# opendilab/DI-engine

Hardware: NVIDIA H100
Metric: learner transitions/sec (GAE+ppo_error fwd+bwd, T=128 x B=4096 per GPU) (higher is better)
Workload: dtype f32

## Files before the change

### di-engine_b200/csrc/colws.cu

```cuda
#include "../../include/b200rl.h"
#include "fused_args.cuh"

namespace b200rl {

constexpr int CW_CW = 8;
constexpr int CW_CT = CW_CW * 32;
constexpr int CW_THREADS = CW_CT + 64;
constexpr int CW_TC = 16;
constexpr int CW_R = CW_CT / CW_TC;
constexpr int CW_MAX_STAGES = 4;
constexpr int CW_RAW_ARR = CW_R * CW_TC * 4;
constexpr int CW_RAW_BYTES = 5 * CW_RAW_ARR;

#define CW_TRACE(slot)                                                                                   \
    do {                                                                                                 \
        if (f.trace) reinterpret_cast<unsigned long long*>(ws + 65536)[blockIdx.x * 32 + (slot)] = gtimer(); \
    } while (0)

struct CwItem {
    long long tile;
    long long q;
};

__host__ __device__ inline int cw_stage_bytes(int N, bool has_pre, bool has_w) {
    return (CW_CT * ((has_pre ? 3 : 2) * N * 4 + 8 + 12 + (has_w ? 4 : 0)) + 127) & ~127;
}

template <int NC, bool GRADS>
__global__ void __launch_bounds__(CW_THREADS, 2) gae_ppo_ws_kernel(FusedArgs f, float* ws, int n_stages) {
    asm volatile("griddepcontrol.launch_dependents;" ::: "memory");
    extern __shared__ __align__(128) unsigned char smem[];
    const PpoArgs& a = f.p;
    const int N = NC ? NC : a.N;
    const int tid = threadIdx.x, wid = tid >> 5, lane = tid & 31;
    const bool has_pre = a.logit_pre != nullptr, has_w = a.weight != nullptr;
    PpoTileLayout L;
    {
        L.logit_bytes = CW_CT * N * 4;
        int o = L.logit_bytes;
        L.off_old = o; o += L.logit_bytes;
        L.off_pre = o; if (has_pre) o += L.logit_bytes;
        L.off_act = o; o += CW_CT * 8;
        L.off_vn = o; o += CW_CT * 4;
        L.off_vo = o; o += CW_CT * 4;
        L.off_adv = 0;
        L.off_ret = o; o += CW_CT * 4;
        L.off_w = o; if (has_w) o += CW_CT * 4;
        L.stage_bytes = (o + 127) & ~127;
        L.tx_bytes = o;
    }
    const int S = n_stages;
    unsigned char* raw = smem + S * L.stage_bytes;
    auto advr = reinterpret_cast<float (*)[CW_R][CW_TC]>(raw + 2 * CW_RAW_BYTES);
    auto fbuf = reinterpret_cast<float (*)[CW_TC]>(reinterpret_cast<unsigned char*>(advr) + CW_MAX_STAGES * CW_RAW_ARR);
    uint64_t* bars = reinterpret_cast<uint64_t*>(reinterpret_cast<unsigned char*>(fbuf) + CW_RAW_ARR);
    uint64_t* full = bars;
    uint64_t* done = bars + CW_MAX_STAGES;
    uint64_t* adv_ready = bars + 2 * CW_MAX_STAGES;

    const long long T = f.T, B = f.B;
    const long long n_tiles = (B + CW_TC - 1) / CW_TC;
    const long long n_chunks = (T + CW_R - 1) / CW_R;
    const bool has_done = f.done != nullptr, has_traj = f.traj != nullptr;

    if (tid == 0) {
        CW_TRACE(0);
        for (int s = 0; s < CW_MAX_STAGES; ++s) {
            mbar_init(&full[s], 32);
            mbar_init(&done[s], CW_CW);
            mbar_init(&adv_ready[s], 1);
        }
        mbar_fence_init();
    }
    asm volatile("griddepcontrol.wait;" ::: "memory");
    __syncthreads();
    if (f.x_mailboxes && blockIdx.x == 0 && wid < 6) {
        XchgArgs x{f.x_mailboxes, f.x_seq, f.x_out_mean, f.x_rank, f.x_world};
        p2p_pipeline_warp(x, wid);
    }

    auto item_valid = [&](const CwItem& it) { return it.tile < n_tiles; };
    auto item_next = [&](CwItem& it) {
        if (++it.q >= n_chunks) {
            it.q = 0;
            it.tile += gridDim.x;
        }
    };
    const CwItem first{(long long)blockIdx.x, 0};
    float acc[6] = {0.f, 0.f, 0.f, 0.f, 0.f, 0.f};

    if (wid == CW_CW) {
        auto rows_of = [&](unsigned char* dst, const void* src, long long t0, long long c0, int esz, int jmin, int W) {
            const int P = CW_TC * esz / 16, Pv = W * esz / 16;
            const unsigned char* g = reinterpret_cast<const unsigned char*>(src) + (t0 * B + c0) * esz;
            const long long rstride = B * esz;
            const int n = CW_R * P;
#pragma unroll 4
            for (int p = lane; p < n; p += 32) {
                const int row = p / P, o = p - row * P;
                if (row >= jmin && o < Pv) cpa16(dst + p * 16, g + row * rstride + o * 16);
            }
        };
        CwItem it = first;
        int s = 0, ph = 0;
        for (int j = 0; item_valid(it); ++j) {
            if (j >= S) mbar_wait(&done[s], (uint32_t)(ph ^ 1));
            if (lane == 0 && j < 6) CW_TRACE(20 + 2 * j);
            const long long c0 = it.tile * CW_TC;
            const long long t0 = T - (it.q + 1) * CW_R;
            const int jmin = t0 < 0 ? (int)-t0 : 0;
            const int W = (int)((B - c0) < CW_TC ? (B - c0) : CW_TC);
            unsigned char* st = smem + s * L.stage_bytes;
            if (jmin == 0 && W == CW_TC && j == 0) {
                const uint32_t sb = smem_u32(st);
                const long long e0 = t0 * B + c0;
                const long long ls = B * N * 4;
                if (N & 1) {
                    warp_copy_rows<4, CW_R, NC>(sb, a.logit_new + e0 * N, ls, N, lane);
                    warp_copy_rows<4, CW_R, NC>(sb + L.off_old, a.logit_old + e0 * N, ls, N, lane);
                    if (has_pre) warp_copy_rows<4, CW_R, NC>(sb + L.off_pre, a.logit_pre + e0 * N, ls, N, lane);
                    warp_copy_rows<4, CW_R, 2>(sb + L.off_act, a.action + e0, B * 8, 2, lane);
                } else {
                    warp_copy_rows<8, CW_R, NC / 2>(sb, a.logit_new + e0 * N, ls, N / 2, lane);
                    warp_copy_rows<8, CW_R, NC / 2>(sb + L.off_old, a.logit_old + e0 * N, ls, N / 2, lane);
                    if (has_pre) warp_copy_rows<8, CW_R, NC / 2>(sb + L.off_pre, a.logit_pre + e0 * N, ls, N / 2, lane);
                    warp_copy_rows<8, CW_R, 1>(sb + L.off_act, a.action + e0, B * 8, 1, lane);
                }
                warp_copy_rows<4, CW_R, 1>(sb + L.off_vn, a.value_new + e0, B * 4, 1, lane);
                warp_copy_rows<4, CW_R, 1>(sb + L.off_vo, a.value_old + e0, B * 4, 1, lane);
                warp_copy_rows<4, CW_R, 1>(sb + L.off_ret, a.ret + e0, B * 4, 1, lane);
                if (has_w) warp_copy_rows<4, CW_R, 1>(sb + L.off_w, a.weight + e0, B * 4, 1, lane);
            } else {
                rows_of(st, a.logit_new, t0, c0, N * 4, jmin, W);
                rows_of(st + L.off_old, a.logit_old, t0, c0, N * 4, jmin, W);
                if (has_pre) rows_of(st + L.off_pre, a.logit_pre, t0, c0, N * 4, jmin, W);
                rows_of(st + L.off_act, a.action, t0, c0, 8, jmin, W);
                rows_of(st + L.off_vn, a.value_new, t0, c0, 4, jmin, W);
                rows_of(st + L.off_vo, a.value_old, t0, c0, 4, jmin, W);
                rows_of(st + L.off_ret, a.ret, t0, c0, 4, jmin, W);
                if (has_w) rows_of(st + L.off_w, a.weight, t0, c0, 4, jmin, W);
            }
            cpa_mbar_arrive(&full[s]);
            if (lane == 0 && j < 6) CW_TRACE(21 + 2 * j);
            if (++s == S) { s = 0; ph ^= 1; }
            item_next(it);
        }
    } else if (wid == CW_CW + 1) {
        auto issue_raw = [&](const CwItem& it, int slot) {
            const long long c0 = it.tile * CW_TC;
            const long long t0 = T - (it.q + 1) * CW_R;
            const int W = (int)((B - c0) < CW_TC ? (B - c0) : CW_TC);
            unsigned char* dst = raw + slot * CW_RAW_BYTES;
#pragma unroll
            for (int k = 0; k < 2; ++k) {
                const int p = lane + 32 * k;
                const int row = p >> 2, o = p & 3;
                if (t0 + row >= 0 && o * 4 < W) {
                    const long long off = (t0 + row) * B + c0 + o * 4;
                    cpa16(dst + p * 16, f.value + off);
                    cpa16(dst + CW_RAW_ARR + p * 16, f.next_value + off);
                    cpa16(dst + 2 * CW_RAW_ARR + p * 16, f.reward + off);
                    if (has_done) cpa16(dst + 3 * CW_RAW_ARR + p * 16, f.done + off);
                    if (has_traj) cpa16(dst + 4 * CW_RAW_ARR + p * 16, f.traj + off);
                }
            }
        };
        CwItem it = first, pf = first;
        for (int k = 0; k < 2; ++k) {
            if (item_valid(pf)) {
                issue_raw(pf, k);
                item_next(pf);
            }
            cpa_commit();
        }
        float carry = 0.f;
        int s = 0, ph = 0;
        for (int j = 0; item_valid(it); ++j) {
            const long long c0 = it.tile * CW_TC;
            const long long t0 = T - (it.q + 1) * CW_R;
            const int slot = j & 1;
            if (it.q == 0) carry = 0.f;
            cpa_wait<1>();
            __syncwarp();
            if (j >= S) mbar_wait(&done[s], (uint32_t)(ph ^ 1));
            float (*ab)[CW_TC] = advr[s];
            const float* rv = reinterpret_cast<const float*>(raw + slot * CW_RAW_BYTES);
            const float* rn = rv + CW_R * CW_TC;
            const float* rr = rn + CW_R * CW_TC;
            const float* rd = rr + CW_R * CW_TC;
            const float* rt = rd + CW_R * CW_TC;
            const int cq = (lane & 3) * 4;
#pragma unroll
            for (int p = 0; p < CW_R / 8; ++p) {
                const int jj = p * 8 + (lane >> 2);
                const long long t = t0 + jj;
                if (t >= 0 && c0 + cq < B) {
                    const int o = jj * CW_TC + cq;
                    const float4 v4 = *reinterpret_cast<const float4*>(rv + o);
                    const float4 n4 = *reinterpret_cast<const float4*>(rn + o);
                    const float4 r4 = *reinterpret_cast<const float4*>(rr + o);
                    const float4 d4 = has_done ? *reinterpret_cast<const float4*>(rd + o) : make_float4(0.f, 0.f, 0.f, 0.f);
                    const float4 t4 = has_traj ? *reinterpret_cast<const float4*>(rt + o) : d4;
                    float vv[4] = {v4.x, v4.y, v4.z, v4.w}, nn[4] = {n4.x, n4.y, n4.z, n4.w};
                    float rw[4] = {r4.x, r4.y, r4.z, r4.w}, dd[4] = {d4.x, d4.y, d4.z, d4.w};
                    float tt[4] = {t4.x, t4.y, t4.z, t4.w};
                    float de[4], fa[4];
                    bool changed = false;
#pragma unroll
                    for (int k = 0; k < 4; ++k) {
                        if (has_done) {
                            changed |= (dd[k] != 0.f);
                            nn[k] = fmul(nn[k], fsub(1.f, dd[k]));
                        }
                        de[k] = fsub(fadd(rw[k], fmul(f.gamma, nn[k])), vv[k]);
                        fa[k] = fmul(f.gl, fsub(1.f, tt[k]));
                    }
                    *reinterpret_cast<float4*>(&ab[jj][cq]) = make_float4(de[0], de[1], de[2], de[3]);
                    *reinterpret_cast<float4*>(&fbuf[jj][cq]) = make_float4(fa[0], fa[1], fa[2], fa[3]);
                    if (changed && f.mask_inplace)
                        *reinterpret_cast<float4*>(f.next_value + t * B + c0 + cq) =
                            make_float4(nn[0], nn[1], nn[2], nn[3]);
                }
            }
            __syncwarp();
            if (item_valid(pf)) {
                issue_raw(pf, slot);
                item_next(pf);
            }
            cpa_commit();
            if (lane < CW_TC && c0 + lane < B) {
                if (t0 >= 0) {
                    float d[CW_R], g[CW_R];
#pragma unroll
                    for (int k = 0; k < CW_R; ++k) {
                        d[k] = ab[CW_R - 1 - k][lane];
                        g[k] = fbuf[CW_R - 1 - k][lane];
                    }
#pragma unroll
                    for (int k = 0; k < CW_R; ++k) {
                        carry = fadd(d[k], fmul(g[k], carry));
                        ab[CW_R - 1 - k][lane] = carry;
                    }
                } else {
                    for (int jj = CW_R - 1; jj >= 0 && t0 + jj >= 0; --jj) {
                        carry = fadd(ab[jj][lane], fmul(fbuf[jj][lane], carry));
                        ab[jj][lane] = carry;
                    }
                }
            }
            __syncwarp();
            if (lane == 0) {
                mbar_arrive(&adv_ready[s]);
                if (j == 0) CW_TRACE(19);
            }
#pragma unroll
            for (int k = 0; k < 2; ++k) {
                const int p = lane + 32 * k;
                const int row = p >> 2, o = (p & 3) * 4;
                if (t0 + row >= 0 && c0 + o < B)
                    stg_stream4(reinterpret_cast<float4*>(a.adv_out + (t0 + row) * B + c0 + o),
                                *reinterpret_cast<const float4*>(&ab[row][o]));
            }
            if (++s == S) { s = 0; ph ^= 1; }
            item_next(it);
        }
        cpa_wait<0>();
    } else {
        PpoUpstream up{0.f, 0.f, 0.f, 0.f, 1.f / (float)a.S};
        if (GRADS) {
            up.g_pol = a.g_policy ? *a.g_policy : 0.f;
            up.g_val = a.g_value ? *a.g_value : 0.f;
            up.g_ent = a.g_entropy ? *a.g_entropy : 0.f;
            up.g_kl = (a.g_kl && has_pre) ? *a.g_kl : 0.f;
            if (a.g_used && blockIdx.x == 0 && tid == 0) {
                a.g_used[0] = up.g_pol; a.g_used[1] = up.g_val; a.g_used[2] = up.g_ent; a.g_used[3] = up.g_kl;
            }
        }
        const int jj = tid / CW_TC, c = tid % CW_TC;
        CwItem it = first;
        int s = 0, ph = 0;
        for (int j = 0; item_valid(it); ++j) {
            const long long c0 = it.tile * CW_TC;
            const long long t = T - (it.q + 1) * CW_R + jj;
            unsigned char* st = smem + s * L.stage_bytes;
            mbar_wait(&full[s], (uint32_t)ph);
            if (tid == 0 && j < 6) CW_TRACE(1 + 3 * j);
            mbar_wait(&adv_ready[s], (uint32_t)ph);
            if (tid == 0 && j < 6) CW_TRACE(2 + 3 * j);
            if (t >= 0 && c0 + c < B) {
                const long long g = t * B + c0 + c;
                float* grow = GRADS ? a.grad_logit + g * N : nullptr;
                float* gval = GRADS ? a.grad_value + g : nullptr;
                ppo_row_compute_to<NC, true, GRADS>(a, L, st, tid, N, advr[s][jj][c], grow, gval, up, acc);
            }
            __syncwarp();
            if (lane == 0) mbar_arrive(&done[s]);
            if (tid == 0 && j < 6) CW_TRACE(3 + 3 * j);
            if (++s == S) { s = 0; ph ^= 1; }
            item_next(it);
        }
    }
    grid_store_partials<6, CW_THREADS>(acc, ws);
}

static size_t cw_smem(int N, bool has_pre, bool has_w, int stages) {
    return (size_t)stages * cw_stage_bytes(N, has_pre, has_w) + 2 * CW_RAW_BYTES + CW_MAX_STAGES * CW_RAW_ARR + CW_RAW_ARR +
           3 * CW_MAX_STAGES * sizeof(uint64_t) + 32;
}

static int cw_pick_stages(const FusedArgs& f) {
    const PpoArgs& a = f.p;
    for (int s = CW_MAX_STAGES; s >= 2; --s)
        if (cw_smem(a.N, a.logit_pre != nullptr, a.weight != nullptr, s) <= 112 * 1024) return s;
    return 0;
}

bool colws_ok(const FusedArgs& f) {
    const PpoArgs& a = f.p;
    const bool al = aligned16(a.logit_new) && aligned16(a.logit_old) && (!a.logit_pre || aligned16(a.logit_pre)) &&
                    aligned16(a.action) && aligned16(a.value_new) && aligned16(a.value_old) && aligned16(a.ret) &&
                    (!a.weight || aligned16(a.weight)) && (!a.grad_logit || aligned16(a.grad_logit)) &&
                    (!a.grad_value || aligned16(a.grad_value)) && aligned16(f.value) && aligned16(f.next_value) &&
                    aligned16(f.reward) && aligned16(a.adv) && (!f.done || aligned16(f.done)) &&
                    (!f.traj || aligned16(f.traj));
    return al && a.N >= 1 && a.N <= 32 && f.T >= 1 && f.B >= 4 && (f.B % 4) == 0 && f.T * f.B == a.S &&
           cw_pick_stages(f) >= 2;
}

template <int NC, bool GRADS>
static int launch_ws(const FusedArgs& f, float* out, float* ws, size_t ws_bytes, cudaStream_t st) {
    const PpoArgs& a = f.p;
    const int stages = cw_pick_stages(f);
    const size_t smem = cw_smem(a.N, a.logit_pre != nullptr, a.weight != nullptr, stages);
    constexpr auto kern = gae_ppo_ws_kernel<NC, GRADS>;
    int sm_count, per_sm;
    if (int rc = resident_ctas<kern>(CW_THREADS, smem, sm_count, per_sm)) return rc;
    const long long n_tiles = (f.B + CW_TC - 1) / CW_TC;
    long long grid = (long long)sm_count * per_sm;
    if (grid > n_tiles) grid = n_tiles;
    if (ws_bytes < WS_MIN_BYTES || !ws_partials_fit((long long)(grid * 6), ws_bytes))
        return B200RL_ERR_WORKSPACE;
    if (int rc = launch_k(kern, (int)grid, CW_THREADS, smem, st, f, ws, stages)) return rc;
    FinalizeArgs fa = ppo_finalize_args(a.S, a.logit_pre != nullptr, (int)grid);
    fa.x.mailboxes = f.x_mailboxes; fa.x.state = f.x_seq; fa.x.out_mean = f.x_out_mean; fa.x.rank = f.x_rank;
    fa.x.world = f.x_world;
    return launch_finalize(ws, out, fa, st);
}

template <bool GRADS>
static int dispatch_ws(const FusedArgs& f, float* out, float* ws, size_t ws_bytes, cudaStream_t st) {
    return with_nc(f.p.N, [&](auto nc) { return launch_ws<nc, GRADS>(f, out, ws, ws_bytes, st); });
}

int launch_colws(const FusedArgs& f, bool grads, float* out, float* ws, size_t ws_bytes, cudaStream_t st) {
    return grads ? dispatch_ws<true>(f, out, ws, ws_bytes, st) : dispatch_ws<false>(f, out, ws, ws_bytes, st);
}

}
```

Before: 17.76 billion.

## Add 32-column tile geometry with one CTA per SM and L2 prefetch of first chunk

Templates the column-tiled warp-specialized GAE+PPO kernel on tile width, adding a 32-column variant (8 rows per chunk, up to 8 stages, one CTA per SM with a 224KB smem budget) picked when B is large enough and at least 6 stages fit. Each CTA also issues bulk L2 prefetches for its first chunk's rows before griddepcontrol.wait, to overlap the first loads with the previous kernel's tail. Tracing is made a compile-time template flag with more slots. The wider tiles are meant to give full 128B row segments and deeper pipelining, at the cost of halving resident CTAs and shortening the per-chunk scan length.

```diff
diff --git a/di-engine_b200/csrc/colws.cu b/di-engine_b200/csrc/colws.cu
--- a/di-engine_b200/csrc/colws.cu
+++ b/di-engine_b200/csrc/colws.cu
@@ -6,15 +6,38 @@
 constexpr int CW_CW = 8;
 constexpr int CW_CT = CW_CW * 32;
 constexpr int CW_THREADS = CW_CT + 64;
-constexpr int CW_TC = 16;
-constexpr int CW_R = CW_CT / CW_TC;
-constexpr int CW_MAX_STAGES = 4;
-constexpr int CW_RAW_ARR = CW_R * CW_TC * 4;
+constexpr int CW_RAW_ARR = CW_CT * 4;
 constexpr int CW_RAW_BYTES = 5 * CW_RAW_ARR;
 
-#define CW_TRACE(slot)                                                                                   \
-    do {                                                                                                 \
-        if (f.trace) reinterpret_cast<unsigned long long*>(ws + 65536)[blockIdx.x * 32 + (slot)] = gtimer(); \
+template <int TC>
+struct CwGeo {
+    static constexpr int R = CW_CT / TC;
+    static constexpr int CPS = TC == 32 ? 1 : 2;
+    static constexpr int MAX_STAGES = TC == 32 ? 8 : 4;
+    static constexpr int SMEM_BUDGET = CPS == 1 ? 224 * 1024 : 112 * 1024;
+    static constexpr int PR = TC / 4;
+};
+
+constexpr int CW_PF = 1;
+__device__ __forceinline__ void prefetch_l2(const void* p, uint32_t bytes) {
+    asm volatile("cp.async.bulk.prefetch.L2.global [%0], %1;" ::"l"(p), "r"(bytes) : "memory");
+}
+
+constexpr int CW_TRACE_CTAS = 512;
+constexpr int CW_TRACE_SLOTS = 64;
+#define CW_TRACE(slot)                                                                                                  \
+    do {                                                                                                                \
+        if (TRACE && blockIdx.x < CW_TRACE_CTAS)                                                                        \
+            reinterpret_cast<unsigned long long*>(ws + 65536)[(blockIdx.x * 2 + (f.trace - 1)) * CW_TRACE_SLOTS + (slot)] = \
+                gtimer();                                                                                               \
+    } while (0)
+__device__ __forceinline__ int cw_trace_k(int j, int nj) { return j < 4 ? j : (j >= nj - 2 && nj > 4) ? 4 + j - (nj - 2) : -1; }
+#define CW_TRACE_CHUNK(first, stride)                           \
+    do {                                                        \
+        if (TRACE) {                                            \
+            const int tk_ = cw_trace_k(j, s_nj);                \
+            if (tk_ >= 0) CW_TRACE((first) + (stride) * tk_);   \
+        }                                                       \
     } while (0)
 
 struct CwItem {
@@ -26,8 +49,10 @@
     return (CW_CT * ((has_pre ? 3 : 2) * N * 4 + 8 + 12 + (has_w ? 4 : 0)) + 127) & ~127;
 }
 
-template <int NC, bool GRADS>
-__global__ void __launch_bounds__(CW_THREADS, 2) gae_ppo_ws_kernel(FusedArgs f, float* ws, int n_stages) {
+template <int NC, bool GRADS, int TC, bool TRACE>
+__global__ void __launch_bounds__(CW_THREADS, CwGeo<TC>::CPS) gae_ppo_ws_kernel(FusedArgs f, float* ws, int n_stages) {
+    using G = CwGeo<TC>;
+    constexpr int R = G::R, PR = G::PR;
     asm volatile("griddepcontrol.launch_dependents;" ::: "memory");
     extern __shared__ __align__(128) unsigned char smem[];
     const PpoArgs& a = f.p;
@@ -51,28 +76,58 @@
     }
     const int S = n_stages;
     unsigned char* raw = smem + S * L.stage_bytes;
-    auto advr = reinterpret_cast<float (*)[CW_R][CW_TC]>(raw + 2 * CW_RAW_BYTES);
-    auto fbuf = reinterpret_cast<float (*)[CW_TC]>(reinterpret_cast<unsigned char*>(advr) + CW_MAX_STAGES * CW_RAW_ARR);
+    auto advr = reinterpret_cast<float (*)[R][TC]>(raw + 2 * CW_RAW_BYTES);
+    auto fbuf = reinterpret_cast<float (*)[TC]>(reinterpret_cast<unsigned char*>(advr) + G::MAX_STAGES * CW_RAW_ARR);
     uint64_t* bars = reinterpret_cast<uint64_t*>(reinterpret_cast<unsigned char*>(fbuf) + CW_RAW_ARR);
     uint64_t* full = bars;
-    uint64_t* done = bars + CW_MAX_STAGES;
-    uint64_t* adv_ready = bars + 2 * CW_MAX_STAGES;
+    uint64_t* done = bars + G::MAX_STAGES;
+    uint64_t* adv_ready = bars + 2 * G::MAX_STAGES;
 
     const long long T = f.T, B = f.B;
-    const long long n_tiles = (B + CW_TC - 1) / CW_TC;
-    const long long n_chunks = (T + CW_R - 1) / CW_R;
+    const long long n_tiles = (B + TC - 1) / TC;
+    const long long n_chunks = (T + R - 1) / R;
     const bool has_done = f.done != nullptr, has_traj = f.traj != nullptr;
+    __shared__ int s_nj;
 
     if (tid == 0) {
         CW_TRACE(0);
-        for (int s = 0; s < CW_MAX_STAGES; ++s) {
+        if (TRACE) s_nj = (int)(n_chunks * ((n_tiles - blockIdx.x + gridDim.x - 1) / gridDim.x));
+        for (int s = 0; s < G::MAX_STAGES; ++s) {
             mbar_init(&full[s], 32);
             mbar_init(&done[s], CW_CW);
             mbar_init(&adv_ready[s], 1);
         }
         mbar_fence_init();
     }
+    {
+        const long long c0 = (long long)blockIdx.x * TC;
+        const long long rows = T < (long long)CW_PF * R ? T : (long long)CW_PF * R;
+        const int W = (int)((B - c0) < TC ? (B - c0) : TC);
+        for (int i = tid; i < 13 * rows; i += CW_THREADS) {
+            const int k = (int)(i / rows);
+            const long long t = T - rows + (i - k * rows);
+            const void* p = nullptr;
+            int esz = 4;
+            switch (k) {
+                case 0: p = a.logit_new; esz = N * 4; break;
+                case 1: p = a.logit_old; esz = N * 4; break;
+                case 2: p = a.logit_pre; esz = N * 4; break;
+                case 3: p = a.action; esz = 8; break;
+                case 4: p = a.value_new; break;
+                case 5: p = a.value_old; break;
+                case 6: p = a.ret; break;
+                case 7: p = a.weight; break;
+                case 8: p = f.value; break;
+                case 9: p = f.next_value; break;
+                case 10: p = f.reward; break;
+                case 11: p = f.done; break;
+                default: p = f.traj; break;
+            }
+            if (p) prefetch_l2(reinterpret_cast<const unsigned char*>(p) + (t * B + c0) * esz, (uint32_t)(W * esz));
+        }
+    }
     asm volatile("griddepcontrol.wait;" ::: "memory");
+    if (tid == 0) CW_TRACE(1);
     __syncthreads();
     if (f.x_mailboxes && blockIdx.x == 0 && wid < 6) {
         XchgArgs x{f.x_mailboxes, f.x_seq, f.x_out_mean, f.x_rank, f.x_world};
@@ -91,10 +146,10 @@
 
     if (wid == CW_CW) {
         auto rows_of = [&](unsigned char* dst, const void* src, long long t0, long long c0, int esz, int jmin, int W) {
-            const int P = CW_TC * esz / 16, Pv = W * esz / 16;
+            const int P = TC * esz / 16, Pv = W * esz / 16;
             const unsigned char* g = reinterpret_cast<const unsigned char*>(src) + (t0 * B + c0) * esz;
             const long long rstride = B * esz;
-            const int n = CW_R * P;
+            const int n = R * P;
 #pragma unroll 4
             for (int p = lane; p < n; p += 32) {
                 const int row = p / P, o = p - row * P;
@@ -105,31 +160,32 @@
         int s = 0, ph = 0;
         for (int j = 0; item_valid(it); ++j) {
             if (j >= S) mbar_wait(&done[s], (uint32_t)(ph ^ 1));
-            if (lane == 0 && j < 6) CW_TRACE(20 + 2 * j);
-            const long long c0 = it.tile * CW_TC;
-            const long long t0 = T - (it.q + 1) * CW_R;
+            if (lane == 0) CW_TRACE_CHUNK(24, 2);
+            const long long c0 = it.tile * TC;
+            const long long t0 = T - (it.q + 1) * R;
             const int jmin = t0 < 0 ? (int)-t0 : 0;
-            const int W = (int)((B - c0) < CW_TC ? (B - c0) : CW_TC);
+            const int W = (int)((B - c0) < TC ? (B - c0) : TC);
             unsigned char* st = smem + s * L.stage_bytes;
-            if (jmin == 0 && W == CW_TC && j == 0) {
+            if (jmin == 0 && W == TC && j == 0) {
                 const uint32_t sb = smem_u32(st);
                 const long long e0 = t0 * B + c0;
                 const long long ls = B * N * 4;
-                if (N & 1) {
-                    warp_copy_rows<4, CW_R, NC>(sb, a.logit_new + e0 * N, ls, N, lane);
-                    warp_copy_rows<4, CW_R, NC>(sb + L.off_old, a.logit_old + e0 * N, ls, N, lane);
-                    if (has_pre) warp_copy_rows<4, CW_R, NC>(sb + L.off_pre, a.logit_pre + e0 * N, ls, N, lane);
-                    warp_copy_rows<4, CW_R, 2>(sb + L.off_act, a.action + e0, B * 8, 2, lane);
+                if (TC == 16 && (N & 1)) {
+                    warp_copy_rows<4, R, NC>(sb, a.logit_new + e0 * N, ls, N, lane);
+                    warp_copy_rows<4, R, NC>(sb + L.off_old, a.logit_old + e0 * N, ls, N, lane);
+                    if (has_pre) warp_copy_rows<4, R, NC>(sb + L.off_pre, a.logit_pre + e0 * N, ls, N, lane);
+                    warp_copy_rows<4, R, 2>(sb + L.off_act, a.action + e0, B * 8, 2, lane);
                 } else {
-                    warp_copy_rows<8, CW_R, NC / 2>(sb, a.logit_new + e0 * N, ls, N / 2, lane);
-                    warp_copy_rows<8, CW_R, NC / 2>(sb + L.off_old, a.logit_old + e0 * N, ls, N / 2, lane);
-                    if (has_pre) warp_copy_rows<8, CW_R, NC / 2>(sb + L.off_pre, a.logit_pre + e0 * N, ls, N / 2, lane);
-                    warp_copy_rows<8, CW_R, 1>(sb + L.off_act, a.action + e0, B * 8, 1, lane);
+                    constexpr int LPG = NC * TC / 32;
+                    warp_copy_rows<8, R, LPG>(sb, a.logit_new + e0 * N, ls, N * TC / 32, lane);
+                    warp_copy_rows<8, R, LPG>(sb + L.off_old, a.logit_old + e0 * N, ls, N * TC / 32, lane);
+                    if (has_pre) warp_copy_rows<8, R, LPG>(sb + L.off_pre, a.logit_pre + e0 * N, ls, N * TC / 32, lane);
+                    warp_copy_rows<8, R, TC / 16>(sb + L.off_act, a.action + e0, B * 8, TC / 16, lane);
                 }
-                warp_copy_rows<4, CW_R, 1>(sb + L.off_vn, a.value_new + e0, B * 4, 1, lane);
-                warp_copy_rows<4, CW_R, 1>(sb + L.off_vo, a.value_old + e0, B * 4, 1, lane);
-                warp_copy_rows<4, CW_R, 1>(sb + L.off_ret, a.ret + e0, B * 4, 1, lane);
-                if (has_w) warp_copy_rows<4, CW_R, 1>(sb + L.off_w, a.weight + e0, B * 4, 1, lane);
+                warp_copy_rows<PR, R, 1>(sb + L.off_vn, a.value_new + e0, B * 4, 1, lane);
+                warp_copy_rows<PR, R, 1>(sb + L.off_vo, a.value_old + e0, B * 4, 1, lane);
+                warp_copy_rows<PR, R, 1>(sb + L.off_ret, a.ret + e0, B * 4, 1, lane);
+                if (has_w) warp_copy_rows<PR, R, 1>(sb + L.off_w, a.weight + e0, B * 4, 1, lane);
             } else {
                 rows_of(st, a.logit_new, t0, c0, N * 4, jmin, W);
                 rows_of(st + L.off_old, a.logit_old, t0, c0, N * 4, jmin, W);
@@ -141,20 +197,20 @@
                 if (has_w) rows_of(st + L.off_w, a.weight, t0, c0, 4, jmin, W);
             }
             cpa_mbar_arrive(&full[s]);
-            if (lane == 0 && j < 6) CW_TRACE(21 + 2 * j);
+            if (lane == 0) CW_TRACE_CHUNK(25, 2);
             if (++s == S) { s = 0; ph ^= 1; }
             item_next(it);
         }
     } else if (wid == CW_CW + 1) {
         auto issue_raw = [&](const CwItem& it, int slot) {
-            const long long c0 = it.tile * CW_TC;
-            const long long t0 = T - (it.q + 1) * CW_R;
-            const int W = (int)((B - c0) < CW_TC ? (B - c0) : CW_TC);
+            const long long c0 = it.tile * TC;
+            const long long t0 = T - (it.q + 1) * R;
+            const int W = (int)((B - c0) < TC ? (B - c0) : TC);
             unsigned char* dst = raw + slot * CW_RAW_BYTES;
 #pragma unroll
             for (int k = 0; k < 2; ++k) {
                 const int p = lane + 32 * k;
-                const int row = p >> 2, o = p & 3;
+                const int row = p / PR, o = p % PR;
                 if (t0 + row >= 0 && o * 4 < W) {
                     const long long off = (t0 + row) * B + c0 + o * 4;
                     cpa16(dst + p * 16, f.value + off);
@@ -176,26 +232,26 @@
         float carry = 0.f;
         int s = 0, ph = 0;
         for (int j = 0; item_valid(it); ++j) {
-            const long long c0 = it.tile * CW_TC;
-            const long long t0 = T - (it.q + 1) * CW_R;
+            const long long c0 = it.tile * TC;
+            const long long t0 = T - (it.q + 1) * R;
             const int slot = j & 1;
             if (it.q == 0) carry = 0.f;
             cpa_wait<1>();
             __syncwarp();
             if (j >= S) mbar_wait(&done[s], (uint32_t)(ph ^ 1));
-            float (*ab)[CW_TC] = advr[s];
+            float (*ab)[TC] = advr[s];
             const float* rv = reinterpret_cast<const float*>(raw + slot * CW_RAW_BYTES);
-            const float* rn = rv + CW_R * CW_TC;
-            const float* rr = rn + CW_R * CW_TC;
-            const float* rd = rr + CW_R * CW_TC;
-            const float* rt = rd + CW_R * CW_TC;
-            const int cq = (lane & 3) * 4;
-#pragma unroll
-            for (int p = 0; p < CW_R / 8; ++p) {
-                const int jj = p * 8 + (lane >> 2);
+            const float* rn = rv + CW_CT;
+            const float* rr = rn + CW_CT;
+            const float* rd = rr + CW_CT;
+            const float* rt = rd + CW_CT;
+#pragma unroll
+            for (int p = 0; p < 2; ++p) {
+                const int q = lane + 32 * p;
+                const int jj = q / PR, cq = (q % PR) * 4;
                 const long long t = t0 + jj;
                 if (t >= 0 && c0 + cq < B) {
-                    const int o = jj * CW_TC + cq;
+                    const int o = jj * TC + cq;
                     const float4 v4 = *reinterpret_cast<const float4*>(rv + o);
                     const float4 n4 = *reinterpret_cast<const float4*>(rn + o);
                     const float4 r4 = *reinterpret_cast<const float4*>(rr + o);
@@ -228,21 +284,21 @@
                 item_next(pf);
             }
             cpa_commit();
-            if (lane < CW_TC && c0 + lane < B) {
+            if (lane < TC && c0 + lane < B) {
                 if (t0 >= 0) {
-                    float d[CW_R], g[CW_R];
-#pragma unroll
-                    for (int k = 0; k < CW_R; ++k) {
-                        d[k] = ab[CW_R - 1 - k][lane];
-                        g[k] = fbuf[CW_R - 1 - k][lane];
+                    float d[R], g[R];
+#pragma unroll
+                    for (int k = 0; k < R; ++k) {
+                        d[k] = ab[R - 1 - k][lane];
+                        g[k] = fbuf[R - 1 - k][lane];
                     }
 #pragma unroll
-                    for (int k = 0; k < CW_R; ++k) {
+                    for (int k = 0; k < R; ++k) {
                         carry = fadd(d[k], fmul(g[k], carry));
-                        ab[CW_R - 1 - k][lane] = carry;
+                        ab[R - 1 - k][lane] = carry;
                     }
                 } else {
-                    for (int jj = CW_R - 1; jj >= 0 && t0 + jj >= 0; --jj) {
+                    for (int jj = R - 1; jj >= 0 && t0 + jj >= 0; --jj) {
                         carry = fadd(ab[jj][lane], fmul(fbuf[jj][lane], carry));
                         ab[jj][lane] = carry;
                     }
@@ -251,12 +307,12 @@
             __syncwarp();
             if (lane == 0) {
                 mbar_arrive(&adv_ready[s]);
-                if (j == 0) CW_TRACE(19);
+                if (j == 0) CW_TRACE(3);
             }
 #pragma unroll
             for (int k = 0; k < 2; ++k) {
                 const int p = lane + 32 * k;
-                const int row = p >> 2, o = (p & 3) * 4;
+                const int row = p / PR, o = (p % PR) * 4;
                 if (t0 + row >= 0 && c0 + o < B)
                     stg_stream4(reinterpret_cast<float4*>(a.adv_out + (t0 + row) * B + c0 + o),
                                 *reinterpret_cast<const float4*>(&ab[row][o]));
@@ -276,17 +332,17 @@
                 a.g_used[0] = up.g_pol; a.g_used[1] = up.g_val; a.g_used[2] = up.g_ent; a.g_used[3] = up.g_kl;
             }
         }
-        const int jj = tid / CW_TC, c = tid % CW_TC;
+        const int jj = tid / TC, c = tid % TC;
         CwItem it = first;
         int s = 0, ph = 0;
         for (int j = 0; item_valid(it); ++j) {
-            const long long c0 = it.tile * CW_TC;
-            const long long t = T - (it.q + 1) * CW_R + jj;
+            const long long c0 = it.tile * TC;
+            const long long t = T - (it.q + 1) * R + jj;
             unsigned char* st = smem + s * L.stage_bytes;
             mbar_wait(&full[s], (uint32_t)ph);
-            if (tid == 0 && j < 6) CW_TRACE(1 + 3 * j);
+            if (tid == 0) CW_TRACE_CHUNK(4, 3);
             mbar_wait(&adv_ready[s], (uint32_t)ph);
-            if (tid == 0 && j < 6) CW_TRACE(2 + 3 * j);
+            if (tid == 0) CW_TRACE_CHUNK(5, 3);
             if (t >= 0 && c0 + c < B) {
                 const long long g = t * B + c0 + c;
                 float* grow = GRADS ? a.grad_logit + g * N : nullptr;
@@ -295,24 +351,37 @@
             }
             __syncwarp();
             if (lane == 0) mbar_arrive(&done[s]);
-            if (tid == 0 && j < 6) CW_TRACE(3 + 3 * j);
+            if (tid == 0) CW_TRACE_CHUNK(6, 3);
             if (++s == S) { s = 0; ph ^= 1; }
             item_next(it);
         }
     }
     grid_store_partials<6, CW_THREADS>(acc, ws);
-}
-
+    if (tid == 0) {
+        CW_TRACE(2);
+        if (TRACE && blockIdx.x < CW_TRACE_CTAS)
+            reinterpret_cast<unsigned long long*>(ws + 65536)[(blockIdx.x * 2 + (f.trace - 1)) * CW_TRACE_SLOTS + 63] = s_nj;
+    }
+}
+
+template <int TC>
 static size_t cw_smem(int N, bool has_pre, bool has_w, int stages) {
-    return (size_t)stages * cw_stage_bytes(N, has_pre, has_w) + 2 * CW_RAW_BYTES + CW_MAX_STAGES * CW_RAW_ARR + CW_RAW_ARR +
-           3 * CW_MAX_STAGES * sizeof(uint64_t) + 32;
-}
-
+    using G = CwGeo<TC>;
+    return (size_t)stages * cw_stage_bytes(N, has_pre, has_w) + 2 * CW_RAW_BYTES + G::MAX_STAGES * CW_RAW_ARR + CW_RAW_ARR +
+           3 * G::MAX_STAGES * sizeof(uint64_t) + 32;
+}
+
+template <int TC>
 static int cw_pick_stages(const FusedArgs& f) {
+    using G = CwGeo<TC>;
     const PpoArgs& a = f.p;
-    for (int s = CW_MAX_STAGES; s >= 2; --s)
-        if (cw_smem(a.N, a.logit_pre != nullptr, a.weight != nullptr, s) <= 112 * 1024) return s;
+    for (int s = G::MAX_STAGES; s >= 2; --s)
+        if (cw_smem<TC>(a.N, a.logit_pre != nullptr, a.weight != nullptr, s) <= (size_t)G::SMEM_BUDGET) return s;
     return 0;
+}
+
+static int cw_pick_tc(const FusedArgs& f) {
+    return (f.B >= 32LL * (NUM_SMS - NUM_SMS / 8) && cw_pick_stages<32>(f) >= 6) ? 32 : 16;
 }
 
 bool colws_ok(const FusedArgs& f) {
@@ -324,23 +393,28 @@
                     aligned16(f.reward) && aligned16(a.adv) && (!f.done || aligned16(f.done)) &&
                     (!f.traj || aligned16(f.traj));
     return al && a.N >= 1 && a.N <= 32 && f.T >= 1 && f.B >= 4 && (f.B % 4) == 0 && f.T * f.B == a.S &&
-           cw_pick_stages(f) >= 2;
-}
-
-template <int NC, bool GRADS>
+           cw_pick_stages<16>(f) >= 2;
+}
+
+template <int NC, bool GRADS, int TC, bool TRACE>
 static int launch_ws(const FusedArgs& f, float* out, float* ws, size_t ws_bytes, cudaStream_t st) {
     const PpoArgs& a = f.p;
-    const int stages = cw_pick_stages(f);
-    const size_t smem = cw_smem(a.N, a.logit_pre != nullptr, a.weight != nullptr, stages);
-    constexpr auto kern = gae_ppo_ws_kernel<NC, GRADS>;
+    const int stages = cw_pick_stages<TC>(f);
+    const size_t smem = cw_smem<TC>(a.N, a.logit_pre != nullptr, a.weight != nullptr, stages);
+    constexpr auto kern = gae_ppo_ws_kernel<NC, GRADS, TC, TRACE>;
     int sm_count, per_sm;
     if (int rc = resident_ctas<kern>(CW_THREADS, smem, sm_count, per_sm)) return rc;
-    const long long n_tiles = (f.B + CW_TC - 1) / CW_TC;
+    const long long n_tiles = (f.B + TC - 1) / TC;
     long long grid = (long long)sm_count * per_sm;
     if (grid > n_tiles) grid = n_tiles;
     if (ws_bytes < WS_MIN_BYTES || !ws_partials_fit((long long)(grid * 6), ws_bytes))
         return B200RL_ERR_WORKSPACE;
-    if (int rc = launch_k(kern, (int)grid, CW_THREADS, smem, st, f, ws, stages)) return rc;
+    FusedArgs fk = f;
+    if (fk.trace) {
+        static unsigned int trace_launches = 0;
+        fk.trace = 1 + (int)(trace_launches++ & 1u);
+    }
+    if (int rc = launch_k(kern, (int)grid, CW_THREADS, smem, st, fk, ws, stages)) return rc;
     FinalizeArgs fa = ppo_finalize_args(a.S, a.logit_pre != nullptr, (int)grid);
     fa.x.mailboxes = f.x_mailboxes; fa.x.state = f.x_seq; fa.x.out_mean = f.x_out_mean; fa.x.rank = f.x_rank;
     fa.x.world = f.x_world;
@@ -349,7 +423,17 @@
 
 template <bool GRADS>
 static int dispatch_ws(const FusedArgs& f, float* out, float* ws, size_t ws_bytes, cudaStream_t st) {
-    return with_nc(f.p.N, [&](auto nc) { return launch_ws<nc, GRADS>(f, out, ws, ws_bytes, st); });
+    const int tc = cw_pick_tc(f);
+    if (f.trace && f.p.N == 6)
+        return tc == 32 ? launch_ws<6, GRADS, 32, true>(f, out, ws, ws_bytes, st)
+                        : launch_ws<6, GRADS, 16, true>(f, out, ws, ws_bytes, st);
+    if (f.trace)
+        return tc == 32 ? launch_ws<0, GRADS, 32, true>(f, out, ws, ws_bytes, st)
+                        : launch_ws<0, GRADS, 16, true>(f, out, ws, ws_bytes, st);
+    return with_nc(f.p.N, [&](auto nc) {
+        return tc == 32 ? launch_ws<nc, GRADS, 32, false>(f, out, ws, ws_bytes, st)
+                        : launch_ws<nc, GRADS, 16, false>(f, out, ws, ws_bytes, st);
+    });
 }
 
 int launch_colws(const FusedArgs& f, bool grads, float* out, float* ws, size_t ws_bytes, cudaStream_t st) {
```

Result: faster. 18.13 billion, median of 6 (+2.1%).
